# rishabhjain16/audio-visual-llm

Measured on AMD Instinct MI355X. Metric: AV-clip train-step samples/sec (clip_whisper -> Llama-2-7B LoRA), whole job, higher is better.
Workload: dtype bf16

## Files before the change

audio-visual-llm_amd/avllm/lib.py:

```python
from __future__ import annotations

import ctypes as C
import os

import torch

_HERE = os.path.dirname(os.path.abspath(__file__))
LIB_PATH = os.environ.get("AVLLM_LIB_PATH") or os.path.join(_HERE, "libavllm.so")

F32, BF16 = 0, 1
ACT_NONE, ACT_GELU, ACT_QUICK_GELU, ACT_SILU = 0, 1, 2, 3
LORA_PAD = 64

i32, i64, f32, vp, sz = C.c_int32, C.c_int64, C.c_float, C.c_void_p, C.c_size_t
fp = C.POINTER(C.c_float)


class GemmDesc(C.Structure):
    _fields_ = [("A", vp), ("B", vp), ("A2", vp), ("B2", vp), ("C", vp), ("bias", vp), ("R", vp),
                ("lda", i64), ("ldb", i64), ("lda2", i64), ("ldb2", i64), ("ldc", i64), ("ldr", i64),
                ("M", i32), ("N", i32), ("K", i32), ("K2", i32), ("dtype", i32), ("out_f32", i32), ("act", i32),
                ("alpha", f32), ("r_mod", i32), ("g_in", i32), ("g_out", i32), ("g_off", i32), ("drop_seed", C.c_uint32), ("drop_p", f32), ("a_drop_seed", C.c_uint32), ("a_drop_p", f32), ("n_valid", i32), ("seed_dev", vp)]


# ... 113 lines not shown
    "avllm_clip_workspace_bytes": ([C.POINTER(Clip), i32], sz),
    "avllm_clip_vision_cls_fwd": ([C.POINTER(Clip), vp, i32, vp, vp, sz, vp], i32),
    "avllm_llama_train_workspace_bytes": ([C.POINTER(Llama), i32, i32], sz),
    "avllm_llama_lora_fwd_loss": ([C.POINTER(Llama), vp, vp, i32, i32, vp, vp, vp, vp, sz, vp], i32),
    "avllm_llama_lora_bwd": ([C.POINTER(Llama), vp, i32, i32, vp, f32, vp, sz, LAYER_CB, vp, vp], i32),
    "avllm_llama_infer_workspace_bytes": ([C.POINTER(Llama), i32, i32], sz),
    "avllm_llama_prefill": ([C.POINTER(Llama), vp, i32, i32, vp, vp, i32, vp, vp, vp, sz, vp], i32),
    "avllm_llama_decode_step": ([C.POINTER(Llama), vp, i32, i32, vp, vp, i32, vp, vp, sz, vp], i32),
    "avllm_llama_decode_step_at": ([C.POINTER(Llama), vp, i32, i32, vp, vp, vp, i32, vp, vp, sz, vp], i32),
    "avllm_llama_decode_is_fused": ([C.POINTER(Llama), i32], i32),
    "avllm_pos_advance": ([vp, i32, vp], i32),
    "avllm_dec_proj": ([C.POINTER(DecProjDesc), vp], i32),
    "avllm_gemm_f8_takes_quantised_output": ([C.POINTER(GemmF8Desc)], i32),
    "avllm_norm_mxq": ([vp, vp, vp, vp, vp, vp, i64, vp, i64, i32, f32, vp], i32),
    "avllm_lora_rank3": ([vp, vp, vp, vp, vp, vp, vp, vp, i32, i32, i32, f32, f32, vp, i32, i32, vp], i32),
    "avllm_gemm_tn_multi": ([vp, i64, i32, vp, vp, vp, vp, vp, vp, vp, i32, i32, i32, f32, f32, vp, i32, i32, vp], i32),
    "avllm_attention_decode": ([vp, i64, vp, vp, vp, i64, i32, i32, i32, i32, vp, i32, f32, i32, i32, vp], i32),
}

EXPORTS = sorted(list(_SIGS) + ["avllm_last_error"])

_lib = None


def load():
    global _lib
    if _lib is not None:
        return _lib
    if not os.path.exists(LIB_PATH):
        raise RuntimeError(f"libavllm.so not found at {LIB_PATH}: run `python build.py` (hipcc, gfx950). "
# ... 62 lines not shown
```

audio-visual-llm_amd/avllm/ops.py:

```python
from __future__ import annotations

import ctypes as C

import torch

from . import lib as L


def _ld(t):
    assert t.stride(-1) == 1, "innermost dimension must be contiguous"
    return t.stride(-2) if t.dim() >= 2 else t.shape[-1]


def gemm(A, B, out=None, bias=None, R=None, A2=None, B2=None, act=L.ACT_NONE, alpha=1.0, out_f32=False,
         r_mod=0, remap=None, M=None, a_drop=None, n_valid=0, drop=None):
    lib = L.load()
    M = A.shape[0] if M is None else M
    N, K = B.shape[0], B.shape[1]
    dt = L.dt_of(A)
    if out is None:
        rows = M if remap is None else (M // remap[0]) * remap[1]
        out = torch.empty(rows, N, device=A.device, dtype=torch.float32 if (out_f32 or dt == L.F32) else A.dtype)
    d = L.GemmDesc()
    d.A, d.B, d.C = L.ptr(A), L.ptr(B), L.ptr(out)
# ... 262 lines not shown
    return outs


def gemm_tn_multi(big, smalls, outs, r, alpha=1.0, seeds=None, p=0.0, shared=False, cols=None, seed_dev=None):
    n = len(smalls)
    arr = lambda ty, vals: (ty * n)(*vals)
    c0 = arr(L.i32, [c[0] for c in cols]) if cols else None
    nc = arr(L.i32, [c[1] for c in cols]) if cols else None
    L.check(L.load().avllm_gemm_tn_multi(L.ptr(big), _ld(big), big.shape[1], arr(L.vp, [L.ptr(t) for t in smalls]), arr(L.i64, [_ld(t) for t in smalls]),
                                         arr(L.vp, [L.ptr(t) for t in outs]), arr(L.i64, [_ld(t) for t in outs]), c0, nc,
                                         arr(C.c_uint32, [(s & 0xFFFFFFFF) for s in (seeds or [0] * n)]), n, r, big.shape[0], alpha, p, seed_dev,
                                         int(shared), L.dt_of(big), L.stream_ptr()))
    return outs


def mx_quantize(x, layout=0):
    lib = L.load()
    R, K = x.shape
    q = torch.empty(R, K, device=x.device, dtype=torch.uint8)
    s = torch.zeros(lib.avllm_mx_scale_bytes(R, K), device=x.device, dtype=torch.uint8)
    L.check(lib.avllm_mx_quantize(L.ptr(x), _ld(x), R, K, L.ptr(q), K, L.ptr(s), layout, L.dt_of(x), L.stream_ptr()))
    return q, s


def gemm_f8(Aq, As, Bq, Bs, out=None, bias=None, R=None, act=L.ACT_NONE, quantised_out=False):
    M, K = Aq.shape
    N = Bq.shape[0]
    d = L.GemmF8Desc()
    d.A, d.SA, d.B, d.SB, d.bias = L.ptr(Aq), L.ptr(As), L.ptr(Bq), L.ptr(Bs), L.ptr(bias)
    d.lda, d.ldb = _ld(Aq), _ld(Bq)
# ... 94 lines not shown
```

audio-visual-llm_amd/csrc/avllm_internal.h:

```cpp
#pragma once
#include <hip/hip_runtime.h>
#include "../../include/avllm.h"

int av_gemm(const avllm_gemm_desc* d, hipStream_t st);
int av_gemm_tn(const void* P, long ldp, int I, const void* Q, long ldq, int J, int M, float* out, long ldo,
               float alpha, int dtype, hipStream_t st, uint32_t drop_seed = 0, float drop_p = 0.f, const uint32_t* seed_dev = nullptr);
int av_layernorm(const void* x, const void* w, const void* b, void* y, long rows, int d, float eps, int dtype, hipStream_t st);
int av_rmsnorm_fwd(const void* x, const void* w, void* y, float* rstd, long rows, int d, float eps, int dtype, hipStream_t st);
int av_rmsnorm_bwd(const void* dy, const void* x, const void* w, const float* rstd, const void* dres_in, void* dx_out,
                   long rows, int d, int dtype, hipStream_t st);
int av_rope(void* x, long ld, long rows, int T, int heads, int hd, int pos0, float theta, int inverse, int dtype, hipStream_t st);
int av_swiglu_fwd(const void* gu, void* h, long M, int F, int dtype, hipStream_t st);
int av_swiglu_bwd(const void* dh, const void* gu, void* dgu, long M, int F, int dtype, hipStream_t st);
bool av_attention_fwd_mxq_ok(int B, int T, int H, int hd, int dtype, int kv_heads);
int av_attention_fwd_mxq(const void* q, const void* k, const void* v, void* oq, long ldoq, void* osc, int B, int T, int H, int hd, long ldq, long ldk,
                         long ldv, float scale, hipStream_t st);
int av_attention_fwd(const void* q, const void* k, const void* v, void* o, float* lse, int B, int Tq, int Tk, int H,
                     int hd, long ldq, long ldk, long ldv, long ldo, float scale, int causal, int dtype, int impl,
                     hipStream_t st, int kv_heads = 0);
int av_attention_bwd(const void* q, const void* k, const void* v, const void* o, const void* dout, const float* lse,
                     void* dq, void* dk, void* dv, float* delta_ws, int B, int T, int H, int hd, long ldq, long ldk,
                     long ldv, long ldo, long lddq, long lddk, long lddv, float scale, int causal, int dtype, int impl,
                     hipStream_t st, int kv_heads = 0, const float* rope_tab = nullptr);
bool av_attention_bwd_fuses_rope(int dtype, int hd, int impl);
// ... 22 lines not shown
                 void* B_pad, void* BT_pad, int dtype, hipStream_t st);
int av_kv_append(const void* k, const void* v, long ld, void* kc, void* vc, int B, int T, int pos0, int Tmax, int d,
                 int dtype, hipStream_t st);
int av_attention_decode(const void* q, long ldq, const void* kc, const void* vc, void* o, long ldo, int B, int H, int hd,
                        int Tk, int Tmax, float scale, int dtype, hipStream_t st, int G = 1);
int av_attention_decode1(const void* q, long ldq, const void* kc, const void* vc, void* o, long ldo, int B, int H, int hd, int Tk, const int* tk_dev,
                         int Tmax, float scale, int dtype, hipStream_t st, int G);
int av_norm_mxq(const void* x, const void* w, const void* b, void* y, float* rstd_out, void* q, long ldq, void* scales, long rows, int d, float eps,
                hipStream_t st);
bool av_lora_batch_supported(int dtype, int R, int nj);
int av_lora_rank3(const void* const* A, const long* lda, const int* K, const void* const* B, const long* ldb, void* const* C, const long* ldc,
                  const uint32_t* seeds, int nj, int M, int R, float alpha, float p, const uint32_t* seed_dev, int shared, int dtype, hipStream_t st);
int av_gemm_tn_multi(const void* Big, long ldb, int NB, const void* const* Small, const long* lds, float* const* out, const long* ldo,
                     const int* col0, const int* ncol, const uint32_t* seeds, int nj, int R, int M, float alpha, float p,
                     const uint32_t* seed_dev, int shared, int dtype, hipStream_t st);
bool av_dec_proj_supported(int dtype, int M, int K, int N, int mode, int hd);
int av_dec_proj(const avllm_dec_proj_desc* d, hipStream_t st);
struct AvRopeScale { float factor = 1.f, low_freq_factor = 1.f, high_freq_factor = 4.f; int orig_ctx = 0; };
int av_rope_table(float* tab, int T, int hd, int pos0, float theta, hipStream_t st, const int* pos_dev = nullptr, AvRopeScale sc = AvRopeScale());
int av_rope_tab(void* x, long ld, long rows, int T, int heads, int hd, const float* tab, int inverse, int dtype, hipStream_t st);
int av_dropout(const void* x, void* y, long rows, int d, uint32_t seed, float p, int dtype, hipStream_t st, const uint32_t* seed_dev = nullptr);
bool av_lora_dx_masked_supported(int dtype, int N, int r, const long* ldt, const long* ldat, int nj, long ldr, long ldo);
int av_lora_dx_masked(const void* const* T, const long* ldt, const void* const* AT, const long* ldat, const uint32_t* seeds, int nj, int r,
                      const void* R, long ldr, void* out, long ldo, int M, int N, float p, const uint32_t* seed_dev, int dtype, hipStream_t st);
int av_mx_quantize(const void* x, long ldx, int R, int K, void* q, long ldq, void* scales, int layout, int dtype, hipStream_t st);
int av_gemm_f8(const avllm_gemm_f8_desc* d, hipStream_t st);
int av_act_residual(const void* x, const void* r, void* y, long n, int act, int dtype, hipStream_t st);
int av_step_advance(avllm_step_state* state, const avllm_schedule* sched, hipStream_t st);
```

audio-visual-llm_amd/csrc/engine.hip:

```cpp
#include "common.h"
#include "avllm_internal.h"

namespace {

struct Bump {
    char* base; size_t cap; size_t off = 0; bool ok = true;
    Bump(void* p, size_t c) : base((char*)p), cap(c) {}
    void* take(size_t bytes) {
        const size_t a = (off + 255) & ~(size_t)255;
        if (a + bytes > cap) { ok = false; off = a + bytes; return base; }
        off = a + bytes;
        return base + a;
    }
};
inline size_t bump_size(const Bump& b) { return ((b.off + 255) & ~(size_t)255) + 256; }

inline avllm_gemm_desc gemm_desc(int dtype, const void* A, long lda, const void* B, long ldb, void* C, long ldc, int M, int N, int K) {
    avllm_gemm_desc g = {};
    g.A = A; g.B = B; g.C = C; g.lda = lda; g.ldb = ldb; g.ldc = ldc; g.M = M; g.N = N; g.K = K;
    g.dtype = dtype; g.alpha = 1.0f;
    return g;
}

inline AvRopeScale llama_rope_scale(const avllm_llama* m) {
// ... 134 lines not shown
inline int llama_kv_heads(const avllm_llama* m);
inline int llama_dkv(const avllm_llama* m);
inline int llama_qw(const avllm_llama* m);
inline int llama_off(const avllm_llama* m, int j);
inline int llama_wid(const avllm_llama* m, int j);
struct LlamaLayerAct {
    void *xn1, *qkv, *att, *tqkv, *to, *h1, *gu;
    float *rstd1, *rstd2, *lse;
};
struct LlamaTrainWs {
    void** resid;
    LlamaLayerAct* act;
    void *xn2, *hmid, *xf, *logits, *xd;
    float *rstd_f, *row_lse, *delta, *rope_tab;
    void *dres, *dxn, *dgu, *dhmid, *dqkv, *datt, *dtqkv, *dto;
    F8Buf f8;
};

void carve_llama_train(const avllm_llama* m, int B, int S, Bump& b, LlamaTrainWs& w, void** resid, LlamaLayerAct* act) {
    const size_t es = av_dtype_size(m->dtype);
    const long M = (long)B * S;
    const int d = m->d, f = m->ffn;
    w.resid = resid; w.act = act;
    for (int l = 0; l <= m->layers; ++l) resid[l] = b.take((size_t)M * d * es);
    for (int l = 0; l < m->layers; ++l) {
        LlamaLayerAct& a = act[l];
        a.xn1 = b.take((size_t)M * d * es);
        a.qkv = b.take((size_t)M * llama_qw(m) * es);
        a.att = b.take((size_t)M * d * es);
        a.tqkv = b.take((size_t)M * 3 * AVLLM_LORA_PAD * es);
// ... 9 lines not shown
    w.xf = b.take((size_t)M * d * es);
    w.logits = b.take((size_t)M * m->vocab * es);
    w.xd = b.take((size_t)M * d * es);
    w.rstd_f = (float*)b.take((size_t)M * 4);
    w.row_lse = (float*)b.take((size_t)M * 4);
    w.delta = (float*)b.take((size_t)B * m->heads * S * 4);
    w.rope_tab = (float*)b.take((size_t)S * (d / m->heads) * 4);
    w.dres = b.take((size_t)M * d * es);
    w.dxn = b.take((size_t)M * d * es);
    w.dgu = b.take((size_t)M * 2 * f * es);
    w.dhmid = b.take((size_t)M * f * es);
    w.dqkv = b.take((size_t)M * llama_qw(m) * es);
    w.datt = b.take((size_t)M * d * es);
    w.dtqkv = b.take((size_t)M * 3 * AVLLM_LORA_PAD * es);
    w.dto = b.take((size_t)M * AVLLM_LORA_PAD * es);
    if (m->fp8) carve_f8(b, w.f8, M, f > d ? f : d);
}

int check_llama(const avllm_llama* m) {
    AV_CHECK_ARG(m && m->layer && m->embed && m->norm_w && m->lm_head, "llama: null model fields");
    AV_CHECK_ARG(m->d % m->heads == 0 && m->d % 64 == 0 && m->ffn % 64 == 0, "llama: d=%d ffn=%d must be multiples of 64", m->d, m->ffn);
    AV_CHECK_ARG(m->layers > 0 && m->layers <= 256, "llama: layers=%d", m->layers);
    AV_CHECK_ARG(m->kv_heads >= 0 && (m->kv_heads == 0 || m->heads % m->kv_heads == 0), "llama: heads=%d kv_heads=%d", m->heads, m->kv_heads);
    return AV_OK;
}
inline int llama_kv_heads(const avllm_llama* m) { return m->kv_heads > 0 ? m->kv_heads : m->heads; }
inline int llama_dkv(const avllm_llama* m) { return llama_kv_heads(m) * (m->d / m->heads); }
inline int llama_qw(const avllm_llama* m) { return m->d + 2 * llama_dkv(m); }
inline int llama_off(const avllm_llama* m, int j) { return j == 0 ? 0 : (j == 1 ? m->d : m->d + llama_dkv(m)); }
inline int llama_wid(const avllm_llama* m, int j) { return j == 0 ? m->d : llama_dkv(m); }
// ... 242 lines not shown
        AV_TRY(av_rmsnorm_bwd(w.dxn, resid[m->layers], m->norm_w, w.rstd_f, nullptr, w.dres, M, d, dt, st));
    }
    for (int l = layer_hi; l >= layer_lo; --l) {
        const avllm_llama_layer& P = m->layer[l];
        LlamaLayerAct& a = act[l];
        AV_CHECK_ARG(P.wqkv_t && P.wo_t && P.wgu_t && P.wdown_t, "llama_lora_bwd: layer %d has no transposed weights", l);
        g = gemm_desc(dt, w.dres, d, P.wdown_t, d, w.dhmid, f, M, f, d);
        AV_TRY(av_gemm(&g, st));
        AV_TRY(av_swiglu_bwd(w.dhmid, a.gu, w.dgu, M, f, dt, st));
        g = gemm_desc(dt, w.dgu, 2 * f, P.wgu_t, 2 * f, w.dxn, d, M, d, 2 * f);
        AV_TRY(av_gemm(&g, st));
        AV_TRY(av_rmsnorm_bwd(w.dxn, a.h1, P.ln2_w, a.rstd2, w.dres, w.dres, M, d, dt, st));
        const avllm_lora_mod& lo = P.lora[3];
        g = gemm_desc(dt, w.dres, d, P.wo_t, d, w.datt, d, M, d, d);
        if (lo.A_pad) {
            AV_TRY(av_gemm_tn(w.dres, d, d, a.to, AVLLM_LORA_PAD, R, M, lo.gB, R, 1.0f, dt, st));
            avllm_gemm_desc gt = gemm_desc(dt, w.dres, d, lo.BT_pad, d, w.dto, AVLLM_LORA_PAD, M, AVLLM_LORA_PAD, d);
            gt.alpha = sc; gt.n_valid = R;
            AV_TRY(av_gemm(&gt, st));
            const void* xin = a.att;
            if (drop && !fuse_drop) { AV_TRY(av_dropout(a.att, w.xd, M, d, m->dropout_seed + 4u * l + 3, m->lora_dropout, dt, st, m->dropout_seed_dev)); xin = w.xd; }
            AV_TRY(av_gemm_tn(w.dto, AVLLM_LORA_PAD, R, xin, d, d, M, lo.gA, d, 1.0f, dt, st, m->dropout_seed + 4u * l + 3,
                              fuse_drop ? m->lora_dropout : 0.f, m->dropout_seed_dev));
            if (!drop) { g.A2 = w.dto; g.lda2 = AVLLM_LORA_PAD; g.B2 = lo.AT_pad; g.ldb2 = lo.ld_at; g.K2 = AVLLM_LORA_PAD; }
        }
        AV_TRY(av_gemm(&g, st));
        if (lo.A_pad && drop) {
            const void* Tp[1] = {w.dto}; const void* Ap[1] = {lo.AT_pad};
            const long lt[1] = {AVLLM_LORA_PAD}, la[1] = {lo.ld_at};
            const uint32_t sd[1] = {m->dropout_seed + 4u * l + 3};
            if (fuse_drop && av_lora_dx_masked_supported(dt, d, R, lt, la, 1, d, d)) {
                AV_TRY(av_lora_dx_masked(Tp, lt, Ap, la, sd, 1, R, w.datt, d, w.datt, d, M, d, m->lora_dropout, m->dropout_seed_dev, dt, st));
            } else {
            avllm_gemm_desc gm = gemm_desc(dt, w.dto, AVLLM_LORA_PAD, lo.AT_pad, lo.ld_at, w.datt, d, M, d, AVLLM_LORA_PAD);
            gm.R = w.datt; gm.ldr = d; gm.drop_seed = m->dropout_seed + 4u * l + 3; gm.drop_p = m->lora_dropout; gm.seed_dev = m->dropout_seed_dev;
            AV_TRY(av_gemm(&gm, st));
            }
        }
        const char* qkv = (const char*)a.qkv;
        char* dqkv = (char*)w.dqkv;
        const bool fuse_rope = av_attention_bwd_fuses_rope(dt, hd, 0);
        AV_TRY(av_attention_bwd(qkv, qkv + (size_t)d * es, qkv + (size_t)(d + dkv) * es, a.att, w.datt, a.lse, dqkv, dqkv + (size_t)d * es,
                                dqkv + (size_t)(d + dkv) * es, w.delta, B, S, H, hd, qw, qw, qw, d, qw, qw, qw,
                                1.0f / sqrtf((float)hd), 1, dt, 0, st, Hkv, fuse_rope ? w.rope_tab : nullptr));
        if (!fuse_rope) AV_TRY(av_rope_tab(dqkv, qw, M, S, H + Hkv, hd, w.rope_tab, 1, dt, st));
        bool any = false, contiguous = true;
        const bool batch_bwd = dt == AV_BF16 && P.lora[0].A_pad && P.lora[1].A_pad && P.lora[2].A_pad && (!drop || fuse_drop) && d % 256 == 0 &&
                               dkv % 256 == 0 && av_lora_batch_supported(dt, R, 3) && !av_knob(AV_KNOB_LORA_UNBATCHED);
        if (batch_bwd) {
            any = true;
            const void* Tq[3]; long ltq[3]; float* gBp[3]; long lgb[3]; int c0[3], nc[3];
            const void* dyp[3]; long ldy[3]; int Kd[3]; const void* BTp[3]; long lbt[3]; void* dtp[3]; long ldt3[3];
            const void* dtc[3]; float* gAp[3]; long lga[3]; uint32_t sd[3];
            for (int j = 0; j < 3; ++j) {
                const avllm_lora_mod& lj = P.lora[j];
                Tq[j] = (char*)a.tqkv + (size_t)j * AVLLM_LORA_PAD * es; ltq[j] = 3 * AVLLM_LORA_PAD; gBp[j] = lj.gB; lgb[j] = R;
                c0[j] = llama_off(m, j); nc[j] = llama_wid(m, j);
                dyp[j] = dqkv + (size_t)llama_off(m, j) * es; ldy[j] = qw; Kd[j] = llama_wid(m, j); BTp[j] = lj.BT_pad; lbt[j] = llama_wid(m, j);
                dtp[j] = (char*)w.dtqkv + (size_t)j * AVLLM_LORA_PAD * es; ldt3[j] = 3 * AVLLM_LORA_PAD; dtc[j] = dtp[j];
                gAp[j] = lj.gA; lga[j] = d; sd[j] = m->dropout_seed + 4u * l + j;
                if (lj.ld_at != 3 * AVLLM_LORA_PAD ||
                    (const char*)lj.AT_pad != (const char*)P.lora[0].AT_pad + (size_t)j * AVLLM_LORA_PAD * es) contiguous = false;
            }
            AV_TRY(av_gemm_tn_multi(dqkv, qw, qw, Tq, ltq, gBp, lgb, c0, nc, nullptr, 3, R, M, 1.0f, 0.f, nullptr, 0, dt, st));
            AV_TRY(av_lora_rank3(dyp, ldy, Kd, BTp, lbt, dtp, ldt3, nullptr, 3, M, R, sc, 0.f, nullptr, 0, dt, st));
            AV_TRY(av_gemm_tn_multi(a.xn1, d, d, dtc, ldt3, gAp, lga, nullptr, nullptr, sd, 3, R, M, 1.0f, drop ? m->lora_dropout : 0.f,
                                    m->dropout_seed_dev, 1, dt, st));
        } else
        for (int j = 0; j < 3; ++j) {
            const avllm_lora_mod& lj = P.lora[j];
            if (!lj.A_pad) { contiguous = false; continue; }
            any = true;
            const char* dy = dqkv + (size_t)llama_off(m, j) * es;
            const int wj = llama_wid(m, j);
            char* dtj = (char*)w.dtqkv + (size_t)j * AVLLM_LORA_PAD * es;
            AV_TRY(av_gemm_tn(dy, qw, wj, (char*)a.tqkv + (size_t)j * AVLLM_LORA_PAD * es, 3 * AVLLM_LORA_PAD, R, M, lj.gB, R, 1.0f, dt, st));
            avllm_gemm_desc gt = gemm_desc(dt, dy, qw, lj.BT_pad, wj, dtj, 3 * AVLLM_LORA_PAD, M, AVLLM_LORA_PAD, wj);
            gt.alpha = sc; gt.n_valid = R;
            AV_TRY(av_gemm(&gt, st));
            const void* xin = a.xn1;
// ... 226 lines not shown
```

audio-visual-llm_amd/csrc/lora_batch.hip:

```cpp
#include "common.h"
#include "avllm_internal.h"

namespace {

constexpr int RK_WAVES = 8;

struct Rank3Args {
    const bf16* A[3]; long lda[3]; int K[3];
    const bf16* B[3]; long ldb[3];
    bf16* C[3]; long ldc[3];
    uint32_t seed[3];
    int nj, M;
    float alpha, p;
    const uint32_t* seed_dev;
};

__device__ __forceinline__ bf16x8 rk_drop(bf16x8 x, uint32_t seed, unsigned long long idx0, uint32_t thr, float sc) {
    float v[8];
#pragma unroll
    for (int j = 0; j < 8; ++j) v[j] = (float)x[j];
    av_mask8(v, seed, idx0, thr, sc);
    bf16x8 r;
#pragma unroll
    for (int j = 0; j < 8; ++j) r[j] = (bf16)v[j];
// ... 182 lines not shown
            for (int i = 0; i < 4; ++i) {
                const int r = fq * 4 + i;
                if (r < a.R) {
                    float* p = SHARED ? a.out[j] + (long)r * a.ldo[j] + n : a.out[j0] + (long)(n - a.col0[j0]) * a.ldo[j0] + r;
                    atomicAdd(p, a.alpha * acc[j][t][i]);
                }
            }
        }
}

int tn_chunks(int M, int want, int& mchunk) {
    int zs = av_cdiv(M, want);
    zs = zs > 32 ? 32 : zs;
    mchunk = av_cdiv(M, zs);
    mchunk = (mchunk + TM_M - 1) / TM_M * TM_M;
    return av_cdiv(M, mchunk);
}

}

bool av_lora_batch_supported(int dtype, int R, int nj) { return dtype == AV_BF16 && R >= 1 && R <= 16 && nj >= 1 && nj <= 3; }

int av_lora_rank3(const void* const* A, const long* lda, const int* K, const void* const* B, const long* ldb, void* const* C, const long* ldc,
                  const uint32_t* seeds, int nj, int M, int R, float alpha, float p, const uint32_t* seed_dev, int shared, int dtype, hipStream_t st) {
    AV_CHECK_ARG(A && lda && K && B && ldb && C && ldc && M > 0, "lora_rank3: null/empty");
    AV_CHECK_ARG(av_lora_batch_supported(dtype, R, nj), "lora_rank3: bf16, rank <= 16 (r=%d), 1..3 adapters (nj=%d)", R, nj);
    AV_CHECK_ARG(p >= 0.f && p < 1.f && (p == 0.f || shared), "lora_rank3: dropout (p=%f) only on the shared-input form", p);
    Rank3Args a = {};
    for (int j = 0; j < nj; ++j) {
        const int ja = shared ? 0 : j;
// ... 41 lines not shown
    const int njk = shared ? nj : 1;
    const size_t lds_bytes = (size_t)njk * TM_M * (TM_BIG + TM_SM);
    static bool attr[64][3] = {};
    int dev = 0;
    AV_HIP(hipGetDevice(&dev));
#define TM_LAUNCH(SH, NJV) do { \
        if (!attr[dev & 63][NJV - 1] && SH) { AV_HIP(hipFuncSetAttribute((const void*)gemm_tn_multi_kernel<SH, NJV>, hipFuncAttributeMaxDynamicSharedMemorySize, (int)lds_bytes)); attr[dev & 63][NJV - 1] = true; } \
        hipLaunchKernelGGL((gemm_tn_multi_kernel<SH, NJV>), grid, dim3(256), lds_bytes, st, a); } while (0)
    if (shared) { if (nj == 3) TM_LAUNCH(true, 3); else if (nj == 2) TM_LAUNCH(true, 2); else TM_LAUNCH(true, 1); }
    else TM_LAUNCH(false, 1);
#undef TM_LAUNCH
    AV_LAUNCH_CHECK();
    return AV_OK;
}

extern "C" int avllm_lora_rank3(const void* const* A, const int64_t* lda, const int32_t* K, const void* const* B, const int64_t* ldb, void* const* C,
                                const int64_t* ldc, const uint32_t* seeds, int32_t nj, int32_t M, int32_t R, float alpha, float p,
                                const uint32_t* seed_dev, int32_t shared, int32_t dtype, void* stream) {
    AV_CHECK_ARG(nj >= 1 && nj <= 3 && lda && K && ldb && ldc, "lora_rank3: nj=%d", nj);
    long la[3], lb[3], lc[3]; int kk[3];
    for (int j = 0; j < nj; ++j) { la[j] = (long)lda[j]; lb[j] = (long)ldb[j]; lc[j] = (long)ldc[j]; kk[j] = K[j]; }
    return av_lora_rank3(A, la, kk, B, lb, C, lc, seeds, nj, M, R, alpha, p, seed_dev, shared, dtype, (hipStream_t)stream);
}

extern "C" int avllm_gemm_tn_multi(const void* Big, int64_t ldb, int32_t NB, const void* const* Small, const int64_t* lds, float* const* out,
                                   const int64_t* ldo, const int32_t* col0, const int32_t* ncol, const uint32_t* seeds, int32_t nj, int32_t R,
                                   int32_t M, float alpha, float p, const uint32_t* seed_dev, int32_t shared, int32_t dtype, void* stream) {
    AV_CHECK_ARG(nj >= 1 && nj <= 3 && lds && ldo, "gemm_tn_multi: nj=%d", nj);
    long ls[3], lo[3]; int c0[3] = {0, 0, 0}, nc[3] = {0, 0, 0};
    for (int j = 0; j < nj; ++j) { ls[j] = (long)lds[j]; lo[j] = (long)ldo[j]; if (col0) c0[j] = col0[j]; if (ncol) nc[j] = ncol[j]; }
    return av_gemm_tn_multi(Big, ldb, NB, Small, ls, out, lo, col0 ? c0 : nullptr, ncol ? nc : nullptr, seeds, nj, R, M, alpha, p, seed_dev, shared,
                            dtype, (hipStream_t)stream);
}
```

audio-visual-llm_amd/csrc/lora_dx.hip:

```cpp
#include "common.h"
#include "avllm_internal.h"

namespace {

constexpr int DX_ROWS = 32, DX_COLS = 128;

struct LoraDxArgs {
    const bf16* T[3]; const bf16* AT[3];
    long ldt[3], ldat[3];
    uint32_t seed[3];
    const bf16* R; bf16* out;
    long ldr, ldo;
    int M, N, nj;
    float p;
    const uint32_t* seed_dev;
};

__device__ __forceinline__ void mask4_add(f32x4& acc, const f32x4 v, uint32_t seed, unsigned long long idx0, uint32_t thr, float sc) {
    const uint32_t h0 = av_pair_hash(seed, idx0 >> 1), h1 = av_pair_hash(seed, (idx0 >> 1) + 1);
    acc[0] += (h0 & 0xffffu) >= thr ? v[0] * sc : 0.f;
    acc[1] += (h0 >> 16) >= thr ? v[1] * sc : 0.f;
    acc[2] += (h1 & 0xffffu) >= thr ? v[2] * sc : 0.f;
    acc[3] += (h1 >> 16) >= thr ? v[3] * sc : 0.f;
}

template <int NJ>
__global__ __launch_bounds__(256) void lora_dx_masked_kernel(LoraDxArgs a) {
    __shared__ __attribute__((aligned(16))) float lds[4 * DX_ROWS * DX_COLS];
    const int lane = threadIdx.x & 63, wave = threadIdx.x >> 6;
    const int fr = lane & 15, fq = lane >> 4;
    const int m0 = (blockIdx.y * 4 + wave) * DX_ROWS, n0 = blockIdx.x * DX_COLS;
    if (m0 >= a.M) return;
    float* cw = lds + wave * DX_ROWS * DX_COLS;
    const uint32_t thr = av_drop_thr(a.p);
    const float sc = av_drop_scale(a.p);
    uint32_t seed[NJ];
#pragma unroll
    for (int j = 0; j < NJ; ++j) seed[j] = av_seed(a.seed_dev, a.seed[j]);
    bf16x8 xa[2][NJ];
#pragma unroll
    for (int rb = 0; rb < 2; ++rb) {
        int m = m0 + rb * 16 + fr;
        m = m < a.M ? m : a.M - 1;
#pragma unroll
        for (int j = 0; j < NJ; ++j) xa[rb][j] = *(const bf16x8*)(a.T[j] + (long)m * a.ldt[j] + fq * 8);
    }
#pragma unroll 2
    for (int ct = 0; ct < DX_COLS / 16; ++ct) {
        bf16x8 wb[NJ];
#pragma unroll
        for (int j = 0; j < NJ; ++j) wb[j] = *(const bf16x8*)(a.AT[j] + (long)(n0 + ct * 16 + fr) * a.ldat[j] + fq * 8);
#pragma unroll
        for (int rb = 0; rb < 2; ++rb) {
            f32x4 acc = {0.f, 0.f, 0.f, 0.f};
            const int row = rb * 16 + fr;
            const unsigned long long idx0 = (unsigned long long)(m0 + row) * a.N + n0 + ct * 16 + 4 * fq;
#pragma unroll
            for (int j = 0; j < NJ; ++j) {
                const f32x4 z = {0.f, 0.f, 0.f, 0.f};
                const f32x4 pj = __builtin_amdgcn_mfma_f32_16x16x32_bf16(wb[j], xa[rb][j], z, 0, 0, 0);
                mask4_add(acc, pj, seed[j], idx0, thr, sc);
            }
            *(f32x4*)(cw + row * DX_COLS + (((ct * 4 + fq) ^ (row & 7)) << 2)) = acc;
        }
    }
    asm volatile("s_waitcnt lgkmcnt(0)" ::: "memory");
#pragma unroll
    for (int i = 0; i < DX_ROWS * (DX_COLS / 8) / 64; ++i) {
        const int c = lane + 64 * i, row = c >> 4, ch = c & 15;
        const int m = m0 + row;
        const f32x4 lo = *(const f32x4*)(cw + row * DX_COLS + (((2 * ch) ^ (row & 7)) << 2));
        const f32x4 hi = *(const f32x4*)(cw + row * DX_COLS + (((2 * ch + 1) ^ (row & 7)) << 2));
        if (m < a.M) {
            float v[8] = {lo[0], lo[1], lo[2], lo[3], hi[0], hi[1], hi[2], hi[3]};
            if (a.R) {
                const bf16x8 r = *(const bf16x8*)(a.R + (long)m * a.ldr + n0 + ch * 8);
#pragma unroll
                for (int q = 0; q < 8; ++q) v[q] += (float)r[q];
            }
            store_f<8>(a.out + (long)m * a.ldo + n0 + ch * 8, v);
        }
    }
}

}

bool av_lora_dx_masked_supported(int dtype, int N, int r, const long* ldt, const long* ldat, int nj, long ldr, long ldo) {
    if (dtype != AV_BF16 || N % DX_COLS != 0 || r > 32 || nj < 1 || nj > 3 || ldr % 8 != 0 || ldo % 8 != 0) return false;
    for (int j = 0; j < nj; ++j)
        if (ldt[j] % 8 != 0 || ldat[j] % 8 != 0 || ldt[j] < 32 || ldat[j] < 32) return false;
    return true;
}

// ... 29 lines not shown
```

include/avllm.h:

```cpp
#ifndef AVLLM_H
#define AVLLM_H
#include <stddef.h>
#include <stdint.h>
#ifdef __cplusplus
extern "C" {
#endif

#define AVLLM_F32 0
#define AVLLM_BF16 1
#define AVLLM_ACT_NONE 0
#define AVLLM_ACT_GELU 1
#define AVLLM_ACT_QUICK_GELU 2
#define AVLLM_ACT_SILU 3
#define AVLLM_LORA_PAD 64

const char* avllm_last_error(void);
int avllm_version(void);


typedef struct avllm_gemm_desc {
    const void* A;  const void* B;
    const void* A2; const void* B2;
    void* C;
    const void* bias;
// ... 16 lines not shown
int avllm_gemm(const avllm_gemm_desc* d, void* stream);
int avllm_set_gemm_variant(int v);
int avllm_set_knob(const char* name, int32_t value);

int avllm_gemm_tn(const void* P, int64_t ldp, int32_t I, const void* Q, int64_t ldq, int32_t J, int32_t M,
                  float* out, int64_t ldo, float alpha, int32_t dtype, void* stream);
int avllm_gemm_tn_drop(const void* P, int64_t ldp, int32_t I, const void* Q, int64_t ldq, int32_t J, int32_t M,
                       float* out, int64_t ldo, float alpha, uint32_t drop_seed, float drop_p, int32_t dtype, void* stream);

int avllm_lora_rank3(const void* const* A, const int64_t* lda, const int32_t* K, const void* const* B, const int64_t* ldb, void* const* C,
                     const int64_t* ldc, const uint32_t* seeds, int32_t nj, int32_t M, int32_t R, float alpha, float p,
                     const uint32_t* seed_dev, int32_t shared, int32_t dtype, void* stream);
int avllm_gemm_tn_multi(const void* Big, int64_t ldb, int32_t NB, const void* const* Small, const int64_t* lds, float* const* out,
                        const int64_t* ldo, const int32_t* col0, const int32_t* ncol, const uint32_t* seeds, int32_t nj, int32_t R,
                        int32_t M, float alpha, float p, const uint32_t* seed_dev, int32_t shared, int32_t dtype, void* stream);

int avllm_lora_dx_masked(const void* const* T, const int64_t* ldt, const void* const* AT, const int64_t* ldat, const uint32_t* seeds,
                         int32_t nj, int32_t r, const void* R, int64_t ldr, void* out, int64_t ldo, int32_t M, int32_t N, float p,
                         const uint32_t* seed_dev, int32_t dtype, void* stream);

size_t avllm_mx_scale_bytes(int32_t R, int32_t K);
int avllm_mx_quantize(const void* x, int64_t ldx, int32_t R, int32_t K, void* q, int64_t ldq, void* scales, int32_t layout, int32_t dtype,
                      void* stream);
typedef struct avllm_gemm_f8_desc {
    const void* A;  const void* SA;
    const void* B;  const void* SB;
    void* C;
    const void* bias;
    const void* R;
    int64_t lda, ldb, ldc, ldr;
// ... 223 lines not shown
```

Measured before the change: 93.22.

## Fuse LoRA dT and gB backward into one pass over the upstream gradient

Adds a lora_dyt kernel that reads the upstream gradient dY once per row slab and computes both the rank-space gradient dT = alpha*dY*B^T and the partial LoRA-B weight gradient T^T*dY. A small reduce kernel then sums the split-M partials. It replaces the separate gemm_tn_multi plus lora_rank3 calls for QKV, and the gemm_tn plus gemm pair for the output projection. It also prefetches the residual in the lora_dx_masked kernel before the main loop. The change adds a workspace allocation and an extra reduction launch, and it accumulates gB with a plain += in the reducer.

```diff
diff --git a/audio-visual-llm_amd/avllm/lib.py b/audio-visual-llm_amd/avllm/lib.py
--- a/audio-visual-llm_amd/avllm/lib.py
+++ b/audio-visual-llm_amd/avllm/lib.py
@@ -151,6 +151,8 @@
     "avllm_gemm_f8_takes_quantised_output": ([C.POINTER(GemmF8Desc)], i32),
     "avllm_norm_mxq": ([vp, vp, vp, vp, vp, vp, i64, vp, i64, i32, f32, vp], i32),
     "avllm_lora_rank3": ([vp, vp, vp, vp, vp, vp, vp, vp, i32, i32, i32, f32, f32, vp, i32, i32, vp], i32),
+    "avllm_lora_dyt_ws_bytes": ([i32, vp, i32], sz),
+    "avllm_lora_dyt": ([vp, i64, vp, vp, vp, vp, vp, vp, vp, vp, vp, vp, i32, i32, i32, f32, vp, sz, i32, vp], i32),
     "avllm_gemm_tn_multi": ([vp, i64, i32, vp, vp, vp, vp, vp, vp, vp, i32, i32, i32, f32, f32, vp, i32, i32, vp], i32),
     "avllm_attention_decode": ([vp, i64, vp, vp, vp, i64, i32, i32, i32, i32, vp, i32, f32, i32, i32, vp], i32),
 }
diff --git a/audio-visual-llm_amd/avllm/ops.py b/audio-visual-llm_amd/avllm/ops.py
--- a/audio-visual-llm_amd/avllm/ops.py
+++ b/audio-visual-llm_amd/avllm/ops.py
@@ -300,6 +300,19 @@
     return outs
 
 
+def lora_dyt(big, cols, BTs, Ts, dts, gBs, r, alpha=1.0):
+    n = len(BTs)
+    arr = lambda ty, vals: (ty * n)(*vals)
+    K = arr(L.i32, [c[1] for c in cols])
+    lib = L.load()
+    ws = torch.empty(max(1, int(lib.avllm_lora_dyt_ws_bytes(n, K, big.shape[0]))), device=big.device, dtype=torch.uint8)
+    L.check(lib.avllm_lora_dyt(L.ptr(big), _ld(big), arr(L.i32, [c[0] for c in cols]), K, arr(L.vp, [L.ptr(t) for t in BTs]),
+                               arr(L.i64, [_ld(t) for t in BTs]), arr(L.vp, [L.ptr(t) for t in Ts]), arr(L.i64, [_ld(t) for t in Ts]),
+                               arr(L.vp, [L.ptr(t) for t in dts]), arr(L.i64, [_ld(t) for t in dts]), arr(L.vp, [L.ptr(t) for t in gBs]),
+                               arr(L.i64, [_ld(t) for t in gBs]), n, big.shape[0], r, alpha, L.ptr(ws), ws.numel(), L.dt_of(big), L.stream_ptr()))
+    return dts, gBs
+
+
 def mx_quantize(x, layout=0):
     lib = L.load()
     R, K = x.shape
diff --git a/audio-visual-llm_amd/csrc/avllm_internal.h b/audio-visual-llm_amd/csrc/avllm_internal.h
--- a/audio-visual-llm_amd/csrc/avllm_internal.h
+++ b/audio-visual-llm_amd/csrc/avllm_internal.h
@@ -60,6 +60,11 @@
 int av_gemm_tn_multi(const void* Big, long ldb, int NB, const void* const* Small, const long* lds, float* const* out, const long* ldo,
                      const int* col0, const int* ncol, const uint32_t* seeds, int nj, int R, int M, float alpha, float p,
                      const uint32_t* seed_dev, int shared, int dtype, hipStream_t st);
+bool av_lora_dyt_supported(int dtype, int R, int nj, const int* K);
+size_t av_lora_dyt_ws_bytes(int nj, const int* K, int M);
+int av_lora_dyt(const void* Big, long ldb, const int* col0, const int* K, const void* const* BT, const long* ldbt, const void* const* T,
+                const long* ldt, void* const* dt, const long* lddt, float* const* gB, const long* ldgb, int nj, int M, int R, float alpha,
+                void* ws, size_t ws_bytes, int dtype, hipStream_t st);
 bool av_dec_proj_supported(int dtype, int M, int K, int N, int mode, int hd);
 int av_dec_proj(const avllm_dec_proj_desc* d, hipStream_t st);
 struct AvRopeScale { float factor = 1.f, low_freq_factor = 1.f, high_freq_factor = 4.f; int orig_ctx = 0; };
diff --git a/audio-visual-llm_amd/csrc/engine.hip b/audio-visual-llm_amd/csrc/engine.hip
--- a/audio-visual-llm_amd/csrc/engine.hip
+++ b/audio-visual-llm_amd/csrc/engine.hip
@@ -172,6 +172,7 @@
     void *xn2, *hmid, *xf, *logits, *xd;
     float *rstd_f, *row_lse, *delta, *rope_tab;
     void *dres, *dxn, *dgu, *dhmid, *dqkv, *datt, *dtqkv, *dto;
+    void* dyt; size_t dyt_bytes;
     F8Buf f8;
 };
 
@@ -211,6 +212,12 @@
     w.datt = b.take((size_t)M * d * es);
     w.dtqkv = b.take((size_t)M * 3 * AVLLM_LORA_PAD * es);
     w.dto = b.take((size_t)M * AVLLM_LORA_PAD * es);
+    {
+        const int kq[3] = {d, llama_dkv(m), llama_dkv(m)}, ko[1] = {d};
+        const size_t q = av_lora_dyt_ws_bytes(3, kq, (int)M), o = av_lora_dyt_ws_bytes(1, ko, (int)M);
+        w.dyt_bytes = q > o ? q : o;
+        w.dyt = b.take(w.dyt_bytes);
+    }
     if (m->fp8) carve_f8(b, w.f8, M, f > d ? f : d);
 }
 
@@ -483,10 +490,17 @@
         const avllm_lora_mod& lo = P.lora[3];
         g = gemm_desc(dt, w.dres, d, P.wo_t, d, w.datt, d, M, d, d);
         if (lo.A_pad) {
-            AV_TRY(av_gemm_tn(w.dres, d, d, a.to, AVLLM_LORA_PAD, R, M, lo.gB, R, 1.0f, dt, st));
-            avllm_gemm_desc gt = gemm_desc(dt, w.dres, d, lo.BT_pad, d, w.dto, AVLLM_LORA_PAD, M, AVLLM_LORA_PAD, d);
-            gt.alpha = sc; gt.n_valid = R;
-            AV_TRY(av_gemm(&gt, st));
+            const int c0[1] = {0}, Ko[1] = {d};
+            if (dt == AV_BF16 && !av_knob(AV_KNOB_LORA_UNBATCHED) && av_lora_dyt_supported(dt, R, 1, Ko)) {
+                const void* BTp[1] = {lo.BT_pad}; const void* Tp[1] = {a.to}; void* dtp[1] = {w.dto}; float* gBp[1] = {lo.gB};
+                const long lbt[1] = {d}, lt[1] = {AVLLM_LORA_PAD}, ldto[1] = {AVLLM_LORA_PAD}, lgb[1] = {R};
+                AV_TRY(av_lora_dyt(w.dres, d, c0, Ko, BTp, lbt, Tp, lt, dtp, ldto, gBp, lgb, 1, M, R, sc, w.dyt, w.dyt_bytes, dt, st));
+            } else {
+                AV_TRY(av_gemm_tn(w.dres, d, d, a.to, AVLLM_LORA_PAD, R, M, lo.gB, R, 1.0f, dt, st));
+                avllm_gemm_desc gt = gemm_desc(dt, w.dres, d, lo.BT_pad, d, w.dto, AVLLM_LORA_PAD, M, AVLLM_LORA_PAD, d);
+                gt.alpha = sc; gt.n_valid = R;
+                AV_TRY(av_gemm(&gt, st));
+            }
             const void* xin = a.att;
             if (drop && !fuse_drop) { AV_TRY(av_dropout(a.att, w.xd, M, d, m->dropout_seed + 4u * l + 3, m->lora_dropout, dt, st, m->dropout_seed_dev)); xin = w.xd; }
             AV_TRY(av_gemm_tn(w.dto, AVLLM_LORA_PAD, R, xin, d, d, M, lo.gA, d, 1.0f, dt, st, m->dropout_seed + 4u * l + 3,
@@ -514,25 +528,25 @@
                                 1.0f / sqrtf((float)hd), 1, dt, 0, st, Hkv, fuse_rope ? w.rope_tab : nullptr));
         if (!fuse_rope) AV_TRY(av_rope_tab(dqkv, qw, M, S, H + Hkv, hd, w.rope_tab, 1, dt, st));
         bool any = false, contiguous = true;
+        const int Kqkv[3] = {d, dkv, dkv};
         const bool batch_bwd = dt == AV_BF16 && P.lora[0].A_pad && P.lora[1].A_pad && P.lora[2].A_pad && (!drop || fuse_drop) && d % 256 == 0 &&
-                               dkv % 256 == 0 && av_lora_batch_supported(dt, R, 3) && !av_knob(AV_KNOB_LORA_UNBATCHED);
+                               dkv % 256 == 0 && av_lora_dyt_supported(dt, R, 3, Kqkv) && !av_knob(AV_KNOB_LORA_UNBATCHED);
         if (batch_bwd) {
             any = true;
             const void* Tq[3]; long ltq[3]; float* gBp[3]; long lgb[3]; int c0[3], nc[3];
-            const void* dyp[3]; long ldy[3]; int Kd[3]; const void* BTp[3]; long lbt[3]; void* dtp[3]; long ldt3[3];
+            const void* BTp[3]; long lbt[3]; void* dtp[3]; long ldt3[3];
             const void* dtc[3]; float* gAp[3]; long lga[3]; uint32_t sd[3];
             for (int j = 0; j < 3; ++j) {
                 const avllm_lora_mod& lj = P.lora[j];
                 Tq[j] = (char*)a.tqkv + (size_t)j * AVLLM_LORA_PAD * es; ltq[j] = 3 * AVLLM_LORA_PAD; gBp[j] = lj.gB; lgb[j] = R;
                 c0[j] = llama_off(m, j); nc[j] = llama_wid(m, j);
-                dyp[j] = dqkv + (size_t)llama_off(m, j) * es; ldy[j] = qw; Kd[j] = llama_wid(m, j); BTp[j] = lj.BT_pad; lbt[j] = llama_wid(m, j);
+                BTp[j] = lj.BT_pad; lbt[j] = llama_wid(m, j);
                 dtp[j] = (char*)w.dtqkv + (size_t)j * AVLLM_LORA_PAD * es; ldt3[j] = 3 * AVLLM_LORA_PAD; dtc[j] = dtp[j];
                 gAp[j] = lj.gA; lga[j] = d; sd[j] = m->dropout_seed + 4u * l + j;
                 if (lj.ld_at != 3 * AVLLM_LORA_PAD ||
                     (const char*)lj.AT_pad != (const char*)P.lora[0].AT_pad + (size_t)j * AVLLM_LORA_PAD * es) contiguous = false;
             }
-            AV_TRY(av_gemm_tn_multi(dqkv, qw, qw, Tq, ltq, gBp, lgb, c0, nc, nullptr, 3, R, M, 1.0f, 0.f, nullptr, 0, dt, st));
-            AV_TRY(av_lora_rank3(dyp, ldy, Kd, BTp, lbt, dtp, ldt3, nullptr, 3, M, R, sc, 0.f, nullptr, 0, dt, st));
+            AV_TRY(av_lora_dyt(dqkv, qw, c0, nc, BTp, lbt, Tq, ltq, dtp, ldt3, gBp, lgb, 3, M, R, sc, w.dyt, w.dyt_bytes, dt, st));
             AV_TRY(av_gemm_tn_multi(a.xn1, d, d, dtc, ldt3, gAp, lga, nullptr, nullptr, sd, 3, R, M, 1.0f, drop ? m->lora_dropout : 0.f,
                                     m->dropout_seed_dev, 1, dt, st));
         } else
diff --git a/audio-visual-llm_amd/csrc/lora_batch.hip b/audio-visual-llm_amd/csrc/lora_batch.hip
--- a/audio-visual-llm_amd/csrc/lora_batch.hip
+++ b/audio-visual-llm_amd/csrc/lora_batch.hip
@@ -220,6 +220,143 @@
     zs = zs > 32 ? 32 : zs;
     mchunk = av_cdiv(M, zs);
     mchunk = (mchunk + TM_M - 1) / TM_M * TM_M;
+    return av_cdiv(M, mchunk);
+}
+
+
+constexpr int DY_ROWS = 32, DY_CBMAX = 512, DY_KS = DY_CBMAX / 32, DY_STRIDE = DY_CBMAX * 2 + 64;
+constexpr int DY_BSTRIDE = DY_CBMAX * 2 + 16;
+
+struct DytArgs {
+    const bf16* Big; long ldb;
+    const bf16* BT[3]; long ldbt[3];
+    const bf16* T[3]; long ldt[3];
+    int col0[3], K[3], gcol0[3];
+    float* pdt;
+    float* pdb;
+    int nj, M, mchunk, NB;
+};
+
+__global__ __launch_bounds__(128) __attribute__((amdgpu_waves_per_eu(2))) void lora_dyt_kernel(DytArgs a) {
+    __shared__ __attribute__((aligned(16))) char big_s[DY_ROWS * DY_STRIDE];
+    __shared__ __attribute__((aligned(16))) char small_s[DY_ROWS * TM_SM];
+    __shared__ __attribute__((aligned(16))) char b_s[16 * DY_BSTRIDE];
+    const int lane = threadIdx.x & 63, g = threadIdx.x >> 6, fr = lane & 15, fq = lane >> 4;
+    const int j = blockIdx.x >> 3, c = blockIdx.x & 7;
+    const int cb = a.K[j] >> 3, ks = cb >> 5, ntw = cb >> 5;
+    const int m_begin = blockIdx.y * a.mchunk, m_end = min(a.M, m_begin + a.mchunk);
+    const bf16* big = a.Big + a.col0[j] + (long)c * cb + fq * 8;
+    for (int e = threadIdx.x; e < 16 * (cb >> 3); e += 128) {
+        const int r = e / (cb >> 3), ch = e % (cb >> 3);
+        *(u32x4*)(b_s + r * DY_BSTRIDE + ch * 16) = *(const u32x4*)(a.BT[j] + (long)r * a.ldbt[j] + (long)c * cb + ch * 8);
+    }
+    f32x4 accb[DY_KS];
+#pragma unroll
+    for (int t = 0; t < DY_KS; ++t) accb[t] = (f32x4){0.f, 0.f, 0.f, 0.f};
+    u32x4 x[DY_KS], ns = {0u, 0u, 0u, 0u};
+    auto fetch = [&](int mb) {
+        const int row = mb + g * 16 + fr;
+        if (row < m_end) {
+            const bf16* p = big + (long)row * a.ldb;
+#pragma unroll
+            for (int s = 0; s < DY_KS; ++s)
+                if (s < ks) x[s] = *(const u32x4*)(p + 32 * s);
+        } else {
+#pragma unroll
+            for (int s = 0; s < DY_KS; ++s) x[s] = (u32x4){0u, 0u, 0u, 0u};
+        }
+        if (g == 0) {
+            const int r2 = mb + (lane >> 1);
+            ns = (u32x4){0u, 0u, 0u, 0u};
+            if (r2 < m_end) ns = *(const u32x4*)(a.T[j] + (long)r2 * a.ldt[j] + (lane & 1) * 8);
+        }
+    };
+    fetch(m_begin);
+    __syncthreads();
+    for (int mb = m_begin; mb < m_end; mb += DY_ROWS) {
+        f32x4 acc = {0.f, 0.f, 0.f, 0.f};
+#pragma unroll
+        for (int s = 0; s < DY_KS; ++s)
+            if (s < ks) {
+                const bf16x8 wb = *(const bf16x8*)(b_s + fr * DY_BSTRIDE + s * 64 + fq * 16);
+                acc = __builtin_amdgcn_mfma_f32_16x16x32_bf16(wb, __builtin_bit_cast(bf16x8, x[s]), acc, 0, 0, 0);
+            }
+        const int row = mb + g * 16 + fr;
+        if (row < m_end) *(f32x4*)(a.pdt + ((long)blockIdx.x * a.M + row) * 16 + fq * 4) = acc;
+        __syncthreads();
+        char* dst = big_s + (g * 16 + fr) * DY_STRIDE + fq * 16;
+#pragma unroll
+        for (int s = 0; s < DY_KS; ++s)
+            if (s < ks) *(u32x4*)(dst + s * 64) = x[s];
+        if (g == 0) *(u32x4*)(small_s + (lane >> 1) * TM_SM + (lane & 1) * 16) = ns;
+        __syncthreads();
+        if (mb + DY_ROWS < m_end) fetch(mb + DY_ROWS);
+        const bf16x8 sa = tn_frag16(small_s, TM_SM, 0, 0, lane);
+#pragma unroll
+        for (int t = 0; t < DY_KS; ++t)
+            if (t < ntw) {
+                const bf16x8 bb = tn_frag16(big_s, DY_STRIDE, 0, (g * ntw + t) * 16, lane);
+                accb[t] = __builtin_amdgcn_mfma_f32_16x16x32_bf16(sa, bb, accb[t], 0, 0, 0);
+            }
+    }
+    float* pb = a.pdb + ((long)blockIdx.y * a.NB + a.gcol0[j] + (long)c * cb) * 16 + fq * 4;
+#pragma unroll
+    for (int t = 0; t < DY_KS; ++t)
+        if (t < ntw) *(f32x4*)(pb + (long)((g * ntw + t) * 16 + fr) * 16) = accb[t];
+}
+
+struct DytReduceArgs {
+    const float* pdt; const float* pdb;
+    bf16* dt[3]; long lddt[3];
+    float* gB[3]; long ldgb[3];
+    int gcol0[3];
+    int nj, M, R, zs, NB;
+    float alpha;
+};
+
+__global__ __launch_bounds__(256) void lora_dyt_reduce_kernel(DytReduceArgs a) {
+    const long i = (long)blockIdx.x * 256 + threadIdx.x;
+    const long ndt = (long)a.nj * a.M * 8;
+    if (i < ndt) {
+        const int q = (int)(i & 7);
+        const long jm = i >> 3;
+        const int j = (int)(jm / a.M), m = (int)(jm % a.M);
+        bf16x8 o;
+#pragma unroll
+        for (int e = 0; e < 8; ++e) o[e] = (bf16)0.f;
+        if (q < 2) {
+            float s[8] = {0.f, 0.f, 0.f, 0.f, 0.f, 0.f, 0.f, 0.f};
+#pragma unroll
+            for (int x = 0; x < RK_WAVES; ++x) {
+                const float* p = a.pdt + ((long)(j * RK_WAVES + x) * a.M + m) * 16 + q * 8;
+                const f32x4 lo = *(const f32x4*)p, hi = *(const f32x4*)(p + 4);
+#pragma unroll
+                for (int e = 0; e < 4; ++e) { s[e] += lo[e]; s[4 + e] += hi[e]; }
+            }
+#pragma unroll
+            for (int e = 0; e < 8; ++e) { s[e] *= a.alpha; o[e] = (bf16)s[e]; }
+        }
+        *(bf16x8*)(a.dt[j] + (long)m * a.lddt[j] + q * 8) = o;
+        return;
+    }
+    const long k = i - ndt;
+    if (k >= (long)a.NB * 16) return;
+    const int n = (int)(k >> 4), r = (int)(k & 15);
+    if (r >= a.R) return;
+    float s = 0.f;
+#pragma unroll 8
+    for (int z = 0; z < a.zs; ++z) s += a.pdb[((long)z * a.NB + n) * 16 + r];
+    const int j = (a.nj > 1 && n >= a.gcol0[1]) + (a.nj > 2 && n >= a.gcol0[2]);
+    float* p = a.gB[j] + (long)(n - a.gcol0[j]) * a.ldgb[j] + r;
+    *p += s;
+}
+
+int dyt_chunks(int nj, int M, int& mchunk) {
+    int zs = av_cdiv(768, 8 * nj);
+    zs = zs > 64 ? 64 : zs;
+    const int slabs = av_cdiv(M, DY_ROWS);
+    zs = zs > slabs ? slabs : zs;
+    mchunk = (av_cdiv(M, zs) + DY_ROWS - 1) / DY_ROWS * DY_ROWS;
     return av_cdiv(M, mchunk);
 }
 
@@ -291,6 +428,52 @@
     return AV_OK;
 }
 
+size_t av_lora_dyt_ws_bytes(int nj, const int* K, int M) {
+    if (nj < 1 || nj > 3 || M <= 0) return 0;
+    long NB = 0;
+    for (int j = 0; j < nj; ++j) NB += K[j];
+    int mchunk = 0;
+    const int zs = dyt_chunks(nj, M, mchunk);
+    return ((size_t)nj * RK_WAVES * M + (size_t)zs * NB) * 16 * sizeof(float);
+}
+
+bool av_lora_dyt_supported(int dtype, int R, int nj, const int* K) {
+    if (!av_lora_batch_supported(dtype, R, nj)) return false;
+    for (int j = 0; j < nj; ++j)
+        if (K[j] <= 0 || K[j] % (32 * RK_WAVES) != 0 || K[j] / RK_WAVES > DY_CBMAX) return false;
+    return true;
+}
+
+int av_lora_dyt(const void* Big, long ldb, const int* col0, const int* K, const void* const* BT, const long* ldbt, const void* const* T,
+                const long* ldt, void* const* dt, const long* lddt, float* const* gB, const long* ldgb, int nj, int M, int R, float alpha,
+                void* ws, size_t ws_bytes, int dtype, hipStream_t st) {
+    AV_CHECK_ARG(Big && col0 && K && BT && ldbt && T && ldt && dt && lddt && gB && ldgb && ws && M > 0 && ldb % 8 == 0, "lora_dyt: null/empty");
+    AV_CHECK_ARG(av_lora_dyt_supported(dtype, R, nj, K), "lora_dyt: bf16, rank <= 16 (r=%d), 1..3 adapters (nj=%d), K %% 256 == 0 and K <= %d",
+                 R, nj, RK_WAVES * DY_CBMAX);
+    AV_CHECK_ARG(ws_bytes >= av_lora_dyt_ws_bytes(nj, K, M), "lora_dyt: workspace %zu < %zu bytes", ws_bytes, av_lora_dyt_ws_bytes(nj, K, M));
+    DytArgs a = {};
+    DytReduceArgs r = {};
+    int nb = 0;
+    for (int j = 0; j < nj; ++j) {
+        AV_CHECK_ARG(BT[j] && T[j] && dt[j] && gB[j], "lora_dyt: null operand %d", j);
+        AV_CHECK_ARG(col0[j] >= 0 && col0[j] % 8 == 0 && ldbt[j] % 8 == 0 && ldt[j] % 8 == 0 && ldt[j] >= 16 && lddt[j] % 8 == 0 && lddt[j] >= 64 &&
+                     ldgb[j] >= R && (uintptr_t)dt[j] % 16 == 0, "lora_dyt: operand %d: 16-byte rows, 64-wide dt outputs", j);
+        a.BT[j] = (const bf16*)BT[j]; a.ldbt[j] = ldbt[j]; a.T[j] = (const bf16*)T[j]; a.ldt[j] = ldt[j];
+        a.col0[j] = col0[j]; a.K[j] = K[j]; a.gcol0[j] = nb; r.gcol0[j] = nb; nb += K[j];
+        r.dt[j] = (bf16*)dt[j]; r.lddt[j] = lddt[j]; r.gB[j] = gB[j]; r.ldgb[j] = ldgb[j];
+    }
+    a.Big = (const bf16*)Big; a.ldb = ldb; a.nj = nj; a.M = M; a.NB = nb;
+    const int zs = dyt_chunks(nj, M, a.mchunk);
+    a.pdt = (float*)ws; a.pdb = a.pdt + (size_t)nj * RK_WAVES * M * 16;
+    hipLaunchKernelGGL(lora_dyt_kernel, dim3(nj * RK_WAVES, zs), dim3(128), 0, st, a);
+    AV_LAUNCH_CHECK();
+    r.pdt = a.pdt; r.pdb = a.pdb; r.nj = nj; r.M = M; r.R = R; r.zs = zs; r.NB = nb; r.alpha = alpha;
+    const long work = (long)nj * M * 8 + (long)nb * 16;
+    hipLaunchKernelGGL(lora_dyt_reduce_kernel, dim3((unsigned)av_cdiv(work, 256)), dim3(256), 0, st, r);
+    AV_LAUNCH_CHECK();
+    return AV_OK;
+}
+
 extern "C" int avllm_lora_rank3(const void* const* A, const int64_t* lda, const int32_t* K, const void* const* B, const int64_t* ldb, void* const* C,
                                 const int64_t* ldc, const uint32_t* seeds, int32_t nj, int32_t M, int32_t R, float alpha, float p,
                                 const uint32_t* seed_dev, int32_t shared, int32_t dtype, void* stream) {
@@ -309,3 +492,19 @@
     return av_gemm_tn_multi(Big, ldb, NB, Small, ls, out, lo, col0 ? c0 : nullptr, ncol ? nc : nullptr, seeds, nj, R, M, alpha, p, seed_dev, shared,
                             dtype, (hipStream_t)stream);
 }
+
+extern "C" size_t avllm_lora_dyt_ws_bytes(int32_t nj, const int32_t* K, int32_t M) {
+    if (nj < 1 || nj > 3 || !K) return 0;
+    int kk[3];
+    for (int j = 0; j < nj; ++j) kk[j] = K[j];
+    return av_lora_dyt_ws_bytes(nj, kk, M);
+}
+
+extern "C" int avllm_lora_dyt(const void* Big, int64_t ldb, const int32_t* col0, const int32_t* K, const void* const* BT, const int64_t* ldbt,
+                              const void* const* T, const int64_t* ldt, void* const* dt, const int64_t* lddt, float* const* gB, const int64_t* ldgb,
+                              int32_t nj, int32_t M, int32_t R, float alpha, void* ws, size_t ws_bytes, int32_t dtype, void* stream) {
+    AV_CHECK_ARG(nj >= 1 && nj <= 3 && col0 && K && ldbt && ldt && lddt && ldgb, "lora_dyt: nj=%d", nj);
+    long lb[3], lt[3], ld[3], lg[3]; int c0[3], kk[3];
+    for (int j = 0; j < nj; ++j) { lb[j] = (long)ldbt[j]; lt[j] = (long)ldt[j]; ld[j] = (long)lddt[j]; lg[j] = (long)ldgb[j]; c0[j] = col0[j]; kk[j] = K[j]; }
+    return av_lora_dyt(Big, (long)ldb, c0, kk, BT, lb, T, lt, dt, ld, gB, lg, nj, M, R, alpha, ws, ws_bytes, dtype, (hipStream_t)stream);
+}
diff --git a/audio-visual-llm_amd/csrc/lora_dx.hip b/audio-visual-llm_amd/csrc/lora_dx.hip
--- a/audio-visual-llm_amd/csrc/lora_dx.hip
+++ b/audio-visual-llm_amd/csrc/lora_dx.hip
@@ -37,6 +37,15 @@
     uint32_t seed[NJ];
 #pragma unroll
     for (int j = 0; j < NJ; ++j) seed[j] = av_seed(a.seed_dev, a.seed[j]);
+    constexpr int CPL = DX_ROWS * (DX_COLS / 8) / 64;
+    bf16x8 rv[CPL];
+#pragma unroll
+    for (int i = 0; i < CPL; ++i) {
+        const int c = lane + 64 * i, m = m0 + (c >> 4);
+#pragma unroll
+        for (int q = 0; q < 8; ++q) rv[i][q] = (bf16)0.f;
+        if (a.R && m < a.M) rv[i] = *(const bf16x8*)(a.R + (long)m * a.ldr + n0 + (c & 15) * 8);
+    }
     bf16x8 xa[2][NJ];
 #pragma unroll
     for (int rb = 0; rb < 2; ++rb) {
@@ -66,7 +75,7 @@
     }
     asm volatile("s_waitcnt lgkmcnt(0)" ::: "memory");
 #pragma unroll
-    for (int i = 0; i < DX_ROWS * (DX_COLS / 8) / 64; ++i) {
+    for (int i = 0; i < CPL; ++i) {
         const int c = lane + 64 * i, row = c >> 4, ch = c & 15;
         const int m = m0 + row;
         const f32x4 lo = *(const f32x4*)(cw + row * DX_COLS + (((2 * ch) ^ (row & 7)) << 2));
@@ -74,9 +83,8 @@
         if (m < a.M) {
             float v[8] = {lo[0], lo[1], lo[2], lo[3], hi[0], hi[1], hi[2], hi[3]};
             if (a.R) {
-                const bf16x8 r = *(const bf16x8*)(a.R + (long)m * a.ldr + n0 + ch * 8);
 #pragma unroll
-                for (int q = 0; q < 8; ++q) v[q] += (float)r[q];
+                for (int q = 0; q < 8; ++q) v[q] += (float)rv[i][q];
             }
             store_f<8>(a.out + (long)m * a.ldo + n0 + ch * 8, v);
         }
diff --git a/include/avllm.h b/include/avllm.h
--- a/include/avllm.h
+++ b/include/avllm.h
@@ -54,6 +54,11 @@
 int avllm_gemm_tn_multi(const void* Big, int64_t ldb, int32_t NB, const void* const* Small, const int64_t* lds, float* const* out,
                         const int64_t* ldo, const int32_t* col0, const int32_t* ncol, const uint32_t* seeds, int32_t nj, int32_t R,
                         int32_t M, float alpha, float p, const uint32_t* seed_dev, int32_t shared, int32_t dtype, void* stream);
+
+size_t avllm_lora_dyt_ws_bytes(int32_t nj, const int32_t* K, int32_t M);
+int avllm_lora_dyt(const void* Big, int64_t ldb, const int32_t* col0, const int32_t* K, const void* const* BT, const int64_t* ldbt,
+                   const void* const* T, const int64_t* ldt, void* const* dt, const int64_t* lddt, float* const* gB, const int64_t* ldgb,
+                   int32_t nj, int32_t M, int32_t R, float alpha, void* ws, size_t ws_bytes, int32_t dtype, void* stream);
 
 int avllm_lora_dx_masked(const void* const* T, const int64_t* ldt, const void* const* AT, const int64_t* ldat, const uint32_t* seeds,
                          int32_t nj, int32_t r, const void* R, int64_t ldr, void* out, int64_t ldo, int32_t M, int32_t N, float p,
```

Result: no change. 93.65, median of 6 (+0.5%).
